# learningmatter-mit/surface-sampling

Measured on AMD Instinct MI355X. Metric: MC energy-evaluations/sec (SrTiO3(001) ~250-atom slabs, 3-model PaiNN ensemble E+F incl. neighbor list), higher is better.
Workload: dtype f32 via fp16x2-split MFMA (3 products), fp32 accumulate; neighbor decisions f64; 1 GPU; SrTiO3(001) PaiNN x3, 256 batched independent chains per GPU (BASELINE configs[3]), 248-272 atoms/chain; chains_per_gpu=256, atoms_per_gpu=66503, edges_per_gpu=2747786, slots_per_gpu=2836316, models=3, streams_per_gpu=2, parallelism=one GPU, no collective

## Files before the change

### include/vssr_eval.h

```cpp
#ifndef VSSR_EVAL_H
#define VSSR_EVAL_H

#include <stddef.h>
#include <stdint.h>

#ifdef __cplusplus
extern "C" {
#endif

#define VSSR_ABI_VERSION 1

enum {
    VSSR_OK = 0,
    VSSR_E_BADARG = -1,
    VSSR_E_DEVICE = -2,
    VSSR_E_CAPACITY = -3,
    VSSR_E_NOMEM = -4,
    VSSR_E_STATE = -5
};

enum {
    VSSR_WANT_ENERGY = 1u,
    VSSR_WANT_FORCES = 2u,
    VSSR_WANT_STD = 4u,
// ... 67 lines not shown
    float maxstep;
} vssr_bfgs_params;
int vssr_batch_relax_bfgs(vssr_handle *h, const vssr_bfgs_params *params, const uint8_t *fixed, uint32_t want,
                          double *pos_out, int32_t *n_steps, uint8_t *converged);

int vssr_batch_traj_configure(vssr_handle *h, int32_t record_interval);
int vssr_batch_traj_read(vssr_handle *h, int32_t cap_records, int32_t *n_records, double *pos, float *forces, double *energy,
                         int32_t *max_records);

typedef struct {
    int32_t max_iter;
    int32_t max_eval;
    double etol, ftol;
    double dmax;
} vssr_cg_params;
int vssr_batch_relax_cg(vssr_handle *h, const vssr_cg_params *params, const uint8_t *fixed, uint32_t want,
                        double *pos_out, int32_t *n_iter, int32_t *n_eval, int32_t *stop_reason);

int vssr_profile_enable(vssr_handle *h, int enable);
int vssr_profile_reset(vssr_handle *h);
int vssr_profile_read(vssr_handle *h, int32_t cap, const char **names, int64_t *launches,
                      double *total_ms, int32_t *n_out);
int vssr_batch_stats(vssr_handle *h, int64_t *n_atoms, int64_t *n_edges, int64_t *n_slots);
int vssr_batch_neighbors(vssr_handle *h, int64_t cap, int32_t *ei, int32_t *ej, int32_t *eS,
                         float *er, int64_t *n_edges);
int vssr_batch_device_results(vssr_handle *h, const float **energy, const float **energy_std);
int vssr_batch_device_results_f64(vssr_handle *h, const double **energy, const double **energy_std);
int vssr_batch_energy_f64(vssr_handle *h, double *energy, double *energy_std, double *energy_models);
int vssr_batch_embedding(vssr_handle *h, int32_t model, float *dst, int64_t cap, int64_t *n_out);
int vssr_batch_saturated(vssr_handle *h, uint8_t *flags, int32_t *n_flagged);
int vssr_batch_stress(vssr_handle *h, double *stress, double *stress_std);
int vssr_device_context(vssr_handle *h, int32_t *device, void **stream, const int32_t **overflow_flag);
int vssr_debug_capacity(vssr_handle *h, int32_t slots_per_atom, int32_t tight, int32_t *n_regrows);
int vssr_batch_relax_counts(vssr_handle *h, int64_t *lockstep_evaluations, int64_t *chain_evaluations);
int vssr_debug_read(vssr_handle *h, const char *name, int32_t model, float *dst, int64_t cap,
                    int64_t *n_out);

typedef struct {
    int32_t nrho, nr;
    double drho, dr, cutoff;
} vssr_eam_grid;
int vssr_eam_create(int32_t device, const vssr_eam_grid *grid, const double *frho, const double *zr, const double *rhor,
                    vssr_handle **out);
int vssr_eam_create_alloy(int32_t device, int32_t n_elem, int32_t fs, const vssr_eam_grid *grid, const double *frho,
                          const double *rhor, const double *z2r, vssr_handle **out);
int vssr_eam_eval_batch(vssr_handle *h, int32_t n_cfg, const int32_t *n_atoms, const int32_t *type, const double *pos,
                        const double *cell, const uint8_t *pbc, uint32_t want, vssr_out *out, double *energy_f64,
                        double *energy_atoms_f64, double *forces_f64);

int vssr_tersoff_create(int32_t device, int32_t n_types, const double *params, vssr_handle **out);
int vssr_tersoff_create_from_text(int32_t device, const char *param_text, int32_t n_species, const char *const *species,
                                  vssr_handle **out);
int vssr_tersoff_eval_batch(vssr_handle *h, int32_t n_cfg, const int32_t *n_atoms,
                            const int32_t *type, const double *pos, const double *cell,
                            const uint8_t *pbc, uint32_t want, vssr_out *out,
                            double *energy_f64 , double *energy_atoms_f64,
                            double *forces_f64);

int vssr_sw_create(int32_t device, int32_t n_types, const double *params, vssr_handle **out);
int vssr_sw_create_from_text(int32_t device, const char *param_text, int32_t n_species, const char *const *species,
                             vssr_handle **out);
int vssr_sw_eval_batch(vssr_handle *h, int32_t n_cfg, const int32_t *n_atoms, const int32_t *type, const double *pos,
                       const double *cell, const uint8_t *pbc, uint32_t want, vssr_out *out, double *energy_f64,
                       double *energy_atoms_f64, double *forces_f64);

typedef struct {
// ... 76 lines not shown
```

### surface-sampling_amd/backend.py

```python

from __future__ import annotations

import ctypes as C
import importlib.util
import os
import sys

import numpy as np

_HERE = os.path.dirname(os.path.abspath(__file__))
LIB_PATH = os.environ.get("VSSR_EVAL_LIB") or os.path.join(_HERE, "libvssr_eval.so")

WANT_ENERGY, WANT_FORCES, WANT_STD, WANT_PER_MODEL, WANT_PER_ATOM = 1, 2, 4, 8, 16
WANT_ALL = WANT_ENERGY | WANT_FORCES | WANT_STD | WANT_PER_MODEL | WANT_PER_ATOM

EXPORTS = (
    "vssr_abi_version", "vssr_create", "vssr_destroy", "vssr_last_error", "vssr_eval", "vssr_eval_batch",
    "vssr_batch_upload", "vssr_batch_set_positions", "vssr_batch_run", "vssr_batch_download",
    "vssr_synchronize", "vssr_profile_enable", "vssr_profile_reset", "vssr_profile_read",
    "vssr_batch_stats", "vssr_batch_neighbors", "vssr_debug_read", "vssr_tersoff_create",
    "vssr_tersoff_eval_batch", "vssr_batch_relax_fire", "vssr_batch_relax_bfgs", "vssr_debug_capacity",
    "vssr_batch_device_results", "vssr_eam_create", "vssr_eam_eval_batch",
    "vssr_tersoff_create_from_text", "vssr_batch_relax_cg", "vssr_batch_saturated",
    "vssr_batch_embedding", "vssr_batch_traj_configure", "vssr_batch_traj_read",
    "vssr_device_context", "vssr_batch_stress", "vssr_batch_energy_f64", "vssr_batch_device_results_f64",
    "vssr_batch_relax_counts", "vssr_sw_create", "vssr_sw_create_from_text", "vssr_sw_eval_batch",
    "vssr_gmm_create", "vssr_gmm_score_rows", "vssr_gmm_score_batch", "vssr_eam_create_alloy",
    "vssr_gmm_fit_create", "vssr_gmm_fit_append_rows", "vssr_gmm_fit_append_batch", "vssr_gmm_fit_clear",
    "vssr_gmm_fit_set_init", "vssr_gmm_fit_run", "vssr_gmm_fit_params", "vssr_gmm_fit_scorer",
    "vssr_cluster_create", "vssr_cluster_append_rows", "vssr_cluster_append_batch", "vssr_cluster_clear", "vssr_cluster_pca",
    "vssr_cluster_pca_params", "vssr_cluster_projected", "vssr_cluster_set_points", "vssr_cluster_linkage",
)


class BackendError(RuntimeError):
    pass


class PainnConfig(C.Structure):
    _fields_ = [
        ("struct_size", C.c_uint32), ("device", C.c_int32), ("n_models", C.c_int32),
        ("weights", C.POINTER(C.POINTER(C.c_float))), ("weights_len", C.c_uint64),
        ("feat_dim", C.c_int32), ("n_rbf", C.c_int32), ("num_conv", C.c_int32), ("n_embed", C.c_int32),
        ("readout_hidden", C.c_int32), ("cutoff", C.c_float), ("excl_vol", C.c_int32),
        ("excl_power", C.c_int32), ("excl_sigma", C.c_float), ("model_units_per_ev", C.c_double),
        ("offset_per_z", C.POINTER(C.c_double)), ("offset_const", C.c_double),
    ]


class FireParams(C.Structure):
    _fields_ = [("max_steps", C.c_int32), ("fmax", C.c_float), ("dt", C.c_float), ("maxstep", C.c_float),
                ("dtmax", C.c_float), ("finc", C.c_float), ("fdec", C.c_float), ("astart", C.c_float),
                ("fa", C.c_float), ("nmin", C.c_int32)]

    @classmethod
    def default(cls, max_steps=20, fmax=0.01):
        return cls(int(max_steps), float(fmax), 0.1, 0.2, 1.0, 1.1, 0.5, 0.1, 0.99, 5)


class EamGrid(C.Structure):
    _fields_ = [("nrho", C.c_int32), ("nr", C.c_int32), ("drho", C.c_double), ("dr", C.c_double), ("cutoff", C.c_double)]


class CgParams(C.Structure):
# ... 139 lines not shown
    L.vssr_eam_eval_batch.argtypes = L.vssr_tersoff_eval_batch.argtypes
    L.vssr_sw_create.restype = C.c_int
    L.vssr_sw_create.argtypes = [C.c_int32, C.c_int32, dp, C.POINTER(vp)]
    L.vssr_sw_create_from_text.restype = C.c_int
    L.vssr_sw_create_from_text.argtypes = [C.c_int32, C.c_char_p, C.c_int32, C.POINTER(C.c_char_p), C.POINTER(vp)]
    L.vssr_sw_eval_batch.restype = C.c_int
    L.vssr_sw_eval_batch.argtypes = L.vssr_tersoff_eval_batch.argtypes
    L.vssr_batch_relax_fire.restype = C.c_int
    L.vssr_batch_relax_fire.argtypes = [vp, C.POINTER(FireParams), u8p, C.c_uint32, dp, ip, u8p]
    L.vssr_batch_relax_bfgs.restype = C.c_int
    L.vssr_batch_relax_bfgs.argtypes = [vp, C.POINTER(BfgsParams), u8p, C.c_uint32, dp, ip, u8p]
    L.vssr_batch_device_results.restype = C.c_int
    L.vssr_batch_device_results.argtypes = [vp, C.POINTER(vp), C.POINTER(vp)]
    L.vssr_batch_device_results_f64.restype = C.c_int
    L.vssr_batch_device_results_f64.argtypes = [vp, C.POINTER(vp), C.POINTER(vp)]
    L.vssr_batch_relax_counts.restype = C.c_int
    L.vssr_batch_relax_counts.argtypes = [vp, i64p, i64p]
    L.vssr_batch_energy_f64.restype = C.c_int
    L.vssr_batch_energy_f64.argtypes = [vp, dp, dp, dp]
    L.vssr_batch_traj_configure.restype = C.c_int
    L.vssr_batch_traj_configure.argtypes = [vp, C.c_int32]
    L.vssr_batch_traj_read.restype = C.c_int
    L.vssr_batch_traj_read.argtypes = [vp, C.c_int32, ip, dp, fp, dp, ip]
    L.vssr_batch_embedding.restype = C.c_int
    L.vssr_batch_embedding.argtypes = [vp, C.c_int32, fp, C.c_int64, i64p]
    L.vssr_batch_saturated.restype = C.c_int
    L.vssr_batch_saturated.argtypes = [vp, u8p, ip]
    L.vssr_batch_stress.restype = C.c_int
    L.vssr_batch_stress.argtypes = [vp, dp, dp]
    L.vssr_device_context.restype = C.c_int
    L.vssr_device_context.argtypes = [vp, ip, C.POINTER(vp), C.POINTER(vp)]
    L.vssr_debug_capacity.restype = C.c_int
    L.vssr_debug_capacity.argtypes = [vp, C.c_int32, C.c_int32, ip]
    L.vssr_gmm_create.restype = C.c_int
    L.vssr_gmm_create.argtypes = [C.POINTER(GmmConfig), C.POINTER(vp)]
    L.vssr_gmm_score_rows.restype = C.c_int
    L.vssr_gmm_score_rows.argtypes = [vp, C.c_int64, dp, dp, dp]
    L.vssr_gmm_score_batch.restype = C.c_int
    L.vssr_gmm_score_batch.argtypes = [vp, vp, C.c_int32, C.c_int32, C.c_int32, dp, dp]
    L.vssr_gmm_fit_create.restype = C.c_int
    L.vssr_gmm_fit_create.argtypes = [C.POINTER(GmmFitConfig), C.POINTER(vp)]
    L.vssr_gmm_fit_append_rows.restype = C.c_int
    L.vssr_gmm_fit_append_rows.argtypes = [vp, C.c_int64, dp]
    L.vssr_gmm_fit_append_batch.restype = C.c_int
    L.vssr_gmm_fit_append_batch.argtypes = [vp, vp, C.c_int32, C.c_int32]
    L.vssr_gmm_fit_clear.restype = C.c_int
    L.vssr_gmm_fit_clear.argtypes = [vp]
    L.vssr_gmm_fit_set_init.restype = C.c_int
    L.vssr_gmm_fit_set_init.argtypes = [vp, dp, dp, dp, C.POINTER(C.c_int32)]
    L.vssr_gmm_fit_run.restype = C.c_int
    L.vssr_gmm_fit_run.argtypes = [vp, C.POINTER(GmmFitResult)]
    L.vssr_gmm_fit_params.restype = C.c_int
    L.vssr_gmm_fit_params.argtypes = [vp, dp, dp, dp, dp]
    L.vssr_gmm_fit_scorer.restype = C.c_int
    L.vssr_gmm_fit_scorer.argtypes = [vp, C.c_double, C.POINTER(vp)]
    L.vssr_cluster_create.restype = C.c_int
    L.vssr_cluster_create.argtypes = [C.POINTER(ClusterConfig), C.POINTER(vp)]
    L.vssr_cluster_append_rows.restype = C.c_int
    L.vssr_cluster_append_rows.argtypes = [vp, C.c_int64, dp]
    L.vssr_cluster_append_batch.restype = C.c_int
    L.vssr_cluster_append_batch.argtypes = [vp, vp, C.c_int32]
    L.vssr_cluster_clear.restype = C.c_int
    L.vssr_cluster_clear.argtypes = [vp]
    L.vssr_cluster_pca.restype = C.c_int
    L.vssr_cluster_pca.argtypes = [vp, C.POINTER(ClusterPcaResult)]
    L.vssr_cluster_pca_params.restype = C.c_int
# ... 614 lines not shown
```

### surface-sampling_amd/csrc/painn_edge_mfma.hip

```cpp
#include "vssr_internal.h"

#ifdef EDGE_PHASE_TIMING
__device__ unsigned long long g_edge_phase[16];
#define EPH_INIT unsigned long long eph_acc[8] = {0, 0, 0, 0, 0, 0, 0, 0}, eph_t = wall_clock64();
#define EPH(k) { __builtin_amdgcn_sched_barrier(0); const unsigned long long eph_n = wall_clock64(); eph_acc[k] += eph_n - eph_t; eph_t = eph_n; __builtin_amdgcn_sched_barrier(0); }
#define EPH_FLUSH(base) if ((threadIdx.x & 63) == 0) { for (int q_ = 0; q_ < 8; ++q_) atomicAdd(&g_edge_phase[(base) + q_], eph_acc[q_]); }
extern "C" int vssr_debug_edge_phases(unsigned long long *out, int reset) {
    if (hipMemcpyFromSymbol(out, HIP_SYMBOL(g_edge_phase), sizeof(unsigned long long) * 16) != hipSuccess) return -1;
    if (reset) { unsigned long long z[16] = {}; if (hipMemcpyToSymbol(HIP_SYMBOL(g_edge_phase), z, sizeof(z)) != hipSuccess) return -1; }
    return 0;
}
#else
#define EPH_INIT
#define EPH(k)
#define EPH_FLUSH(base)
#endif

#ifndef SUB16_WAVES
#define SUB16_WAVES 12
#endif

namespace vssr {

typedef float f32x4 __attribute__((ext_vector_type(4)));
// ... 98 lines not shown
                split2(Wd[(size_t)row * 20 + kq + 4 * t], p2);
                wh[t] = p2[0]; wl[t] = p2[1];
            }
            split2(bd[row], bp);
            const unsigned bias = kq == 1 ? bp[1] : kq == 3 ? 0u : bp[0];
            const unsigned a1[8] = {wh[0], wh[1], wh[2], wh[3], wh[4], bias, wl[0], wl[1]};
            const unsigned a2[8] = {wl[2], wl[3], wl[4], wh[4], wh[0], wh[1], wh[2], wh[3]};
            unsigned *o = dst + ((size_t)row * 4 + kq) * 8;
            for (int q = 0; q < 4; ++q) {
                o[q] = a1[2 * q] | (a1[2 * q + 1] << 16);
                o[4 + q] = a2[2 * q] | (a2[2 * q + 1] << 16);
            }
        }
}

#ifndef STAGE_BATCH
#define STAGE_BATCH 4
#endif

template <int N> struct FeatVec { typedef float type __attribute__((ext_vector_type(N))); };
struct FeatVec1 {
    float v;
    __device__ __forceinline__ float operator[](int) const { return v; }
};
template <> struct FeatVec<1> { typedef FeatVec1 type; };

template <int NF>
struct EdgeGeo {
    static_assert(NF == 4 || NF == 2 || NF == 1, "16-, 8- or 4-feature slices");
    static constexpr int FS = 4 * NF;
    static constexpr int NSLICE = F / FS;
    static constexpr int NSEC = 3;
    static constexpr int NT = NF == 4 ? 3 : NF == 2 ? 2 : 1;
    static constexpr int NSEG = 6;
    static constexpr int ROW = NSEG * FS + 4;
    static constexpr int ROWB = FS * 4 + 4;
    __host__ __device__ static constexpr int row_section(int T, int i) {
        return NF == 4 ? T : NF == 1 ? ((i & 3) < 3 ? (i & 3) : -1) : (2 * T + ((i & 3) >> 1) < 3 ? 2 * T + ((i & 3) >> 1) : -1);
    }
    __host__ __device__ static constexpr int row_feature(int i) { return NF == 4 ? i : NF == 1 ? (i >> 2) : 2 * (i >> 2) + (i & 1); }
};
template <int NF> __device__ __forceinline__ constexpr int sec_tile(int sec) { return NF == 4 ? sec : NF == 1 ? 0 : sec >> 1; }
template <int NF> __device__ __forceinline__ constexpr int sec_reg(int sec, int r) { return NF == 4 ? r : NF == 1 ? sec : 2 * (sec & 1) + r; }

template <int NF, bool SLDS>
size_t edge_fwd_lds_bytes_t(int max_atoms) {
    return sizeof(float) * ((size_t)max_atoms * (EdgeGeo<NF>::ROW + (SLDS ? EdgeGeo<NF>::FS : 0)) + 4);
}

typedef float f32x2v __attribute__((ext_vector_type(2)));
#if defined(__HIP_DEVICE_COMPILE__)
typedef __attribute__((address_space(3))) const float lds_cfloat;
__device__ __forceinline__ lds_cfloat *lds_base(const float *p) { return (lds_cfloat *)p; }
__device__ __forceinline__ lds_cfloat *lds_row(lds_cfloat *base, int row, int row_floats) {
    return base + __umul24((unsigned)row, (unsigned)row_floats);
}
__device__ __forceinline__ f32x4 lds_read4(lds_cfloat *p) { return *reinterpret_cast<__attribute__((address_space(3))) const f32x4 *>(p); }
__device__ __forceinline__ f32x2v lds_read2(lds_cfloat *p) { return *reinterpret_cast<__attribute__((address_space(3))) const f32x2v *>(p); }
#else
typedef const float lds_cfloat;
__host__ __device__ inline lds_cfloat *lds_base(const float *p) { return p; }
__host__ __device__ inline lds_cfloat *lds_row(lds_cfloat *base, int row, int row_floats) { return base + row * row_floats; }
__host__ __device__ inline f32x4 lds_read4(lds_cfloat *p) { return *reinterpret_cast<const f32x4 *>(p); }
__host__ __device__ inline f32x2v lds_read2(lds_cfloat *p) { return *reinterpret_cast<const f32x2v *>(p); }
#endif

__device__ __forceinline__ float quad_sum(float x) {
    x += __builtin_bit_cast(float, __builtin_amdgcn_update_dpp(0, __builtin_bit_cast(int, x), 0xB1, 0xF, 0xF, true));
// ... 84 lines not shown
template <bool ALIASED> struct EdgeOut { typedef float *__restrict__ ptr; };
template <> struct EdgeOut<true> { typedef float *ptr; };

template <int NF, bool SLDS, int WAVES, bool SUB = false>
__global__ void __launch_bounds__(64 * WAVES) __attribute__((amdgpu_waves_per_eu((SUB && NF == 4) ? WAVES / 4 : 4, (SUB && NF == 4) ? WAVES / 4 : 4)))
k_edge_fwd_mfma(int N, int l, const ModelW *__restrict__ MW, GraphView G, const int *__restrict__ counters,
                int zero_slot, int n_models, int max_atoms, const int *__restrict__ list, int n_list,
                const float *__restrict__ s_in, const float *__restrict__ v_in, const float *__restrict__ phi,
                typename EdgeOut<SUB>::ptr s_msg, typename EdgeOut<SUB>::ptr v_msg, const int4 *__restrict__ bundle_tab,
                const int *__restrict__ n_entries_tab, int pass, int chunk_max) {
    using LY = EdgeGeo<NF>;
    constexpr int FS = LY::FS, NSLICE = LY::NSLICE, NT = LY::NT, EDGE_THREADS = 64 * WAVES;
    static_assert(!SUB || !SLDS, "the sub-range form takes its residuals from memory");
    extern __shared__ __attribute__((aligned(16))) float tile[];
    if (counters[2]) return;
    int t;
    const int b = chain_of_workgroup(G, list, n_list, NSLICE * n_models, t);
    if (b < 0) return;
    const int fs = t % NSLICE, m = t / NSLICE;
    const int a0 = G.cfg_start[b], Nc = G.cfg_start[b + 1] - a0;
    const size_t mN = (size_t)m * N;
    const int tid = threadIdx.x;
    int lo = 0, ns = Nc;
    if constexpr (SUB) {
        if (pass >= sub_passes(Nc, chunk_max)) return;
        const int chunk = sub_chunk(Nc, chunk_max);
        lo = pass * chunk;
        ns = min(chunk, Nc - lo);
    }
    const float *res_s = (SUB && pass) ? s_msg : s_in, *res_v = (SUB && pass) ? v_msg : v_in;

    float *s_tile = tile + (size_t)max_atoms * LY::ROW;
    {
        constexpr int Q4 = FS / 4;
        constexpr int PER_ATOM = (LY::NSEG + (SLDS ? 1 : 0)) * Q4;
        const int total = ns * PER_ATOM;
        if constexpr (SUB) {
            for (int k = tid; k < LY::ROW; k += EDGE_THREADS) tile[(size_t)ns * LY::ROW + k] = 0.f;
        }
        auto src_of = [&](int idx) -> const float * {
            int atom = idx / PER_ATOM, rem = idx - atom * PER_ATOM, seg = rem / Q4, q4 = rem % Q4;
            const size_t ga = mN + a0 + lo + atom;
            if (seg == LY::NSEG) return s_in + ga * F + fs * FS + q4 * 4;
            if (seg < 3) return phi + ga * F3 + seg * F + fs * FS + q4 * 4;
            return v_in + (ga * 3 + (seg - 3)) * F + fs * FS + q4 * 4;
        };
        auto put = [&](int idx, const float4 &val) {
            int atom = idx / PER_ATOM, rem = idx - atom * PER_ATOM, seg = rem / Q4, q4 = rem % Q4;
            if (seg == LY::NSEG) {
                *reinterpret_cast<float4 *>(s_tile + atom * FS + q4 * 4) = val;
            } else {
                float *dst = tile + atom * LY::ROW + (q4 * 4) * LY::NSEG + seg;
                dst[0] = val.x; dst[LY::NSEG] = val.y; dst[2 * LY::NSEG] = val.z; dst[3 * LY::NSEG] = val.w;
            }
        };
        for (int base = tid; base < total; base += STAGE_BATCH * EDGE_THREADS) {
            float4 v4[STAGE_BATCH];
#pragma unroll
            for (int u = 0; u < STAGE_BATCH; ++u) {
                const int idx = min(base + u * EDGE_THREADS, total - 1);
                v4[u] = *reinterpret_cast<const float4 *>(src_of(idx));
            }
#pragma unroll
            for (int u = 0; u < STAGE_BATCH; ++u)
                if (base + u * EDGE_THREADS < total) put(base + u * EDGE_THREADS, v4[u]);
        }
    }
    __syncthreads();

    const int lane = tid & 63, wave = tid >> 6, p = lane & 15, fq = lane >> 4, e = p & 3;
    const LayerW &W = MW[m].layer[l];
    u32x4 wA[NT][2];
#pragma unroll
    for (int T = 0; T < NT; ++T) {
        const int sec = LY::row_section(T, p);
        const int row = max(sec, 0) * F + fs * FS + LY::row_feature(p);
        const u32x4 *wsrc = reinterpret_cast<const u32x4 *>(W.wd16) + ((size_t)row * 4 + fq) * 2;
#pragma unroll
        for (int i3 = 0; i3 < 2; ++i3) wA[T][i3] = sec < 0 ? (u32x4){0u, 0u, 0u, 0u} : gload_u32x4(wsrc + i3);
    }

    BundleWalk<EDGE_THREADS / 64> bw;
    int n_entries = Nc;
    if constexpr (SUB) {
        if (pass) n_entries = n_entries_tab[(size_t)(pass - 1) * G.n_cfg + b];
    }
    bw.init((SUB ? bundle_tab : G.bundle) + a0, n_entries, __builtin_amdgcn_readfirstlane(wave), p >> 2);
    if (bw.nj == 0) return;
#ifdef ABL_STAGE_ONLY
    if (bw.nj > 0) return;
#endif
    float ds[NF], dvx[NF], dvy[NF], dvz[NF];
#pragma unroll
    for (int r = 0; r < NF; ++r) { ds[r] = 0.f; dvx[r] = 0.f; dvy[r] = 0.f; dvz[r] = 0.f; }
    const int fcol = fs * FS + NF * fq;
    typedef typename FeatVec<NF>::type fres;
    fres sres_cur, sres_nxt, vres_cur[SUB ? 3 : 1];
    auto load_residual = [&](int cc) {
        return *reinterpret_cast<const fres *>(res_s + (mN + a0 + min(max(cc, 0), Nc - 1)) * F + fcol);
    };
    auto load_residual_v = [&](int cc, int x) {
        return *reinterpret_cast<const fres *>(res_v + ((mN + a0 + min(max(cc, 0), Nc - 1)) * 3 + x) * F + fcol);
    };
    if (!SLDS) { sres_cur = load_residual(bw.cur.x); sres_nxt = load_residual(bw.nxt.x); }
    if constexpr (SUB) {
#pragma unroll
        for (int x = 0; x < 3; ++x) vres_cur[x] = load_residual_v(bw.cur.x, x);
    }

    const u32x4 *rho_lane = reinterpret_cast<const u32x4 *>(G.rho16) + fq * 4 + e;
    const int zero_quad = (zero_slot + 1) / 4 - 1;

    u32x4 rq[2][2];
    auto fetch = [&](int buf, int quad_first_slot, bool valid) {
#ifdef ABL_TABLE_L2
        const u32x4 *rp = rho_lane + (size_t)(valid ? ((quad_first_slot >> 2) & 511) : zero_quad) * 32;
#else
        const u32x4 *rp = rho_lane + (size_t)(unsigned)(valid ? (quad_first_slot >> 2) : zero_quad) * 32;
#endif
        rq[buf][0] = rp[0]; rq[buf][1] = rp[16];
    };
    {
        bool v0, v1;
        const int q0 = bw.quad_ahead(0, v0), q1 = bw.quad_ahead(1, v1);
        fetch(0, q0, v0);
        __builtin_amdgcn_sched_barrier(0);
        fetch(1, q1, v1);
    }

    auto flush_bundle = [&]() {
        quad_sum_n<NF>(ds); quad_sum_n<NF>(dvx); quad_sum_n<NF>(dvy); quad_sum_n<NF>(dvz);
        const int c = bw.cur.x;
        if (e == 0 && c >= 0) {
            const size_t ga = mN + a0 + c;
            float so[NF], xo[NF], yo[NF], zo[NF];
            const float *sr = s_tile + c * FS + NF * fq;
            const float *vc = tile + c * LY::ROW + (NF * fq) * LY::NSEG;
#pragma unroll
            for (int r = 0; r < NF; ++r) {
                so[r] = ds[r] + (SLDS ? sr[r] : sres_cur[r]);
                xo[r] = dvx[r] + (SUB ? vres_cur[0][r] : vc[r * LY::NSEG + 3]);
                yo[r] = dvy[r] + (SUB ? vres_cur[SUB ? 1 : 0][r] : vc[r * LY::NSEG + 4]);
                zo[r] = dvz[r] + (SUB ? vres_cur[SUB ? 2 : 0][r] : vc[r * LY::NSEG + 5]);
            }
            store_feat<NF>(s_msg + ga * F + fcol, so);
            store_feat<NF>(v_msg + (ga * 3 + 0) * F + fcol, xo);
            store_feat<NF>(v_msg + (ga * 3 + 1) * F + fcol, yo);
            store_feat<NF>(v_msg + (ga * 3 + 2) * F + fcol, zo);
        }
#pragma unroll
        for (int r = 0; r < NF; ++r) { ds[r] = 0.f; dvx[r] = 0.f; dvy[r] = 0.f; dvz[r] = 0.f; }
    };

    lds_cfloat *trow = lds_base(tile) + (NF * fq) * LY::NSEG;
    EPH_INIT
    EPH(0)
    while (bw.j < bw.nj) {
#pragma unroll
        for (int ph = 0; ph < 2; ++ph) {
            arrival_fence(rq[ph][0], rq[ph][1]);
            EPH(1)
#ifdef ABL_LDS_BCAST
            const int jn = (int)(rq[ph][0][3] >> 16) & 1;
#else
            int jn = (int)rq[ph][1][3];
            if constexpr (SUB) {
                const unsigned jl = (unsigned)(jn - lo);
                jn = jl < (unsigned)ns ? (int)jl : ns;
            }
#endif
            if (bw.t == bw.Lc) {
                flush_bundle();
                bw.advance();
                if (!SLDS) {
                    sres_cur = sres_nxt;
                    __builtin_amdgcn_sched_barrier(0);
                    sres_nxt = load_residual(bw.nxt.x);
                    if constexpr (SUB) {
#pragma unroll
                        for (int x = 0; x < 3; ++x) vres_cur[x] = load_residual_v(bw.cur.x, x);
                    }
                }
                EPH(2)
            }
            float tv[NF * LY::NSEG];
            {
                if constexpr ((NF * LY::NSEG) % 4 == 0) {
                    lds_cfloat *row = lds_row(trow, jn, LY::ROW);
#pragma unroll
                    for (int q = 0; q < NF * LY::NSEG / 4; ++q) {
                        const f32x4 t4 = lds_read4(row + 4 * q);
                        tv[4 * q] = t4[0]; tv[4 * q + 1] = t4[1]; tv[4 * q + 2] = t4[2]; tv[4 * q + 3] = t4[3];
                    }
                } else {
                    lds_cfloat *row = lds_row(trow, jn, LY::ROW);
#pragma unroll
                    for (int q = 0; q < NF * LY::NSEG / 2; ++q) {
                        const f32x2v t2 = lds_read2(row + 2 * q);
                        tv[2 * q] = t2[0]; tv[2 * q + 1] = t2[1];
                    }
                }
            }
            float ux, uy, uz, invd_unused;
            slot_scalars(take_u(rq[ph][1][2]), ux, uy, uz, invd_unused);
            u32x4 rb2 = dense_b2(rq[ph][0], rq[ph][1]);
            mfma_pre_fence(rq[ph][0], rb2);
            EPH(3)
            f32x4 acc[NT];
            {
                const u32x4 (*wp[NT])[2], *bp1[NT], *bp2[NT];
#pragma unroll
                for (int s2 = 0; s2 < NT; ++s2) { wp[s2] = &wA[s2]; bp1[s2] = &rq[ph][0]; bp2[s2] = &rb2; }
                filter_tiles_dense<NT>(wp, bp1, bp2, acc);
            }
            __builtin_amdgcn_sched_barrier(0);
            EPH(4)
            auto message = [&](int r) {
                const float *tr = tv + r * LY::NSEG;
                const float wa = acc[sec_tile<NF>(0)][sec_reg<NF>(0, r)], wb = acc[sec_tile<NF>(1)][sec_reg<NF>(1, r)],
                            wc = acc[sec_tile<NF>(2)][sec_reg<NF>(2, r)];
                ds[r] = fmaf(tr[1], wb, ds[r]);
                const float mc = tr[2] * wc, ma = tr[0] * wa;
                dvx[r] = fmaf(mc, ux, dvx[r]); dvy[r] = fmaf(mc, uy, dvy[r]); dvz[r] = fmaf(mc, uz, dvz[r]);
                dvx[r] = fmaf(ma, tr[3], dvx[r]);
                dvy[r] = fmaf(ma, tr[4], dvy[r]);
                dvz[r] = fmaf(ma, tr[5], dvz[r]);
            };
            message(0);
            bool nv;
            int nq = bw.quad_ahead(2, nv);
            mfma_load_fence(nq, ds[0], dvx[0], dvy[0]);
            EPH(5)
            fetch(ph, nq, nv);
            __builtin_amdgcn_sched_barrier(0);
#ifdef ABL_HALF_VALU
#pragma unroll
            for (int r = 1; r < NF / 2; ++r) message(r);
#else
#pragma unroll
            for (int r = 1; r < NF; ++r) message(r);
#endif
            ++bw.t;
            EPH(6)
        }
    }
    EPH_FLUSH(0)
}

template <int NF, int WAVES>
constexpr int cen_floats() { return WAVES * 4 * 4 * 6 * NF; }
template <int NF, int WAVES>
#ifdef ABL_LDS_FORCE
size_t edge_bwd_lds_bytes_t(int max_atoms) { return sizeof(float) * ((size_t)max_atoms * EdgeGeo<NF>::ROWB + cen_floats<NF, WAVES>()) + 24 * (size_t)max_atoms + 32; }
#else
size_t edge_bwd_lds_bytes_t(int max_atoms) { return sizeof(float) * ((size_t)max_atoms * EdgeGeo<NF>::ROWB + cen_floats<NF, WAVES>()); }
#endif

template <int NF, bool FIRST, int WAVES, bool SUB = false>
__global__ void __launch_bounds__(64 * WAVES) __attribute__((amdgpu_waves_per_eu(2, 2)))
// ... 342 lines not shown
            }
            ++bw.t;
            EPH(7)
        }
    }
    EPH_FLUSH(8)
#ifdef ABL_LDS_FORCE
    __syncthreads();
    {
        unsigned long long *dst = reinterpret_cast<unsigned long long *>(gb) + (size_t)3 * a0;
        for (int i = tid; i < 3 * Nc; i += BWD_THREADS) dst[i] = facc[i];
    }
#endif
}



int edge_mfma_init(vssr_handle *h) {
#define SET_LDS(K) VSSR_HIP(h, hipFuncSetAttribute((const void *)(K), hipFuncAttributeMaxDynamicSharedMemorySize, 160 * 1024))
    SET_LDS((k_edge_fwd_mfma<4, true, 16>)); SET_LDS((k_edge_fwd_mfma<4, false, 16>)); SET_LDS((k_edge_fwd_mfma<2, false, 16>)); SET_LDS((k_edge_fwd_mfma<2, false, 16, true>)); SET_LDS((k_edge_fwd_mfma<4, false, SUB16_WAVES, true>));
    SET_LDS((k_edge_fwd_mfma<4, true, 8>)); SET_LDS((k_edge_fwd_mfma<4, true, 4>)); SET_LDS((k_edge_fwd_mfma<1, false, 16>));
    SET_LDS((k_edge_bwd_mfma<1, true, 4>)); SET_LDS((k_edge_bwd_mfma<1, false, 4>));
    SET_LDS((k_edge_bwd_mfma<1, true, 8>)); SET_LDS((k_edge_bwd_mfma<1, false, 8>));
    SET_LDS((k_edge_bwd_mfma<4, true, 4>)); SET_LDS((k_edge_bwd_mfma<4, false, 4>));
    SET_LDS((k_edge_bwd_mfma<2, true, 4>)); SET_LDS((k_edge_bwd_mfma<2, false, 4>));
    SET_LDS((k_edge_bwd_mfma<4, true, 8>)); SET_LDS((k_edge_bwd_mfma<4, false, 8>));
    SET_LDS((k_edge_bwd_mfma<4, true, 8, true>)); SET_LDS((k_edge_bwd_mfma<4, false, 8, true>));
    SET_LDS((k_edge_bwd_mfma<2, true, 8>)); SET_LDS((k_edge_bwd_mfma<2, false, 8>));
#undef SET_LDS
    return VSSR_OK;
}

int edge_class_of(int n_atoms) {
    if (edge_fwd_lds_bytes_t<4, true>(n_atoms) <= 160 * 1024) return EDGE_CLASS_FS16;
    if (edge_fwd_lds_bytes_t<4, false>(n_atoms) <= 160 * 1024) return EDGE_CLASS_FS16M;
    if (edge_fwd_lds_bytes_t<2, false>(n_atoms) <= 160 * 1024) return EDGE_CLASS_FS8;
    if (edge_fwd_lds_bytes_t<1, false>(n_atoms) <= 160 * 1024) return EDGE_CLASS_FS4;
    return EDGE_CLASS_GATHER;
}
int edge_bclass_of(int n_atoms) {
    const int fwd = edge_class_of(n_atoms);
    if (fwd == EDGE_CLASS_GATHER) return EDGE_BCLASS_GATHER;
    if (edge_bwd_lds_bytes_t<4, 8>(n_atoms) <= 160 * 1024) return EDGE_BCLASS_FS16;
    if (edge_bwd_lds_bytes_t<2, 8>(n_atoms) <= 160 * 1024) return EDGE_BCLASS_FS8;
    return EDGE_BCLASS_FS4;
}
int edge_class_groups(int bcls) { return edge_bclass_slices(bcls); }
static_assert(edge_bclass_slices(EDGE_BCLASS_FS16) == EdgeGeo<4>::NSLICE && edge_bclass_slices(EDGE_BCLASS_FS8) == EdgeGeo<2>::NSLICE &&
              edge_bclass_slices(EDGE_BCLASS_FS4) == EdgeGeo<1>::NSLICE, "slices per reverse class");

void launch_edge_bwd_mfma(hipStream_t st, int cls, int N, const int *list, int n_list, int M, int l, int layer_first, int max_atoms,
                          const ModelW *MW, const GraphView &G, const int *counters, int zero_slot,
                          const float *v_in, const float *phi, const float *sbar_msg, const float *vbar_msg,
                          float *phibar, float *vbar_in, float *gbar, long long gbar_stride, int n_groups, int group_off, int rec,
                          const int4 *bundle_sub, int sub_chunk) {
    if (n_list <= 0) return;
    if (cls == EDGE_BCLASS_FS16P) {
        const int chunk_max = sub_chunk, passes = sub_passes(max_atoms, chunk_max), staged = min(chunk_max, max_atoms) + 1;
        const int *n_entries = reinterpret_cast<const int *>(bundle_sub + (size_t)SUB_MAX_PASSES * N);
        for (int pass = 0; pass < passes; ++pass) {
#define LAUNCH_BWD_SUB(FIRST)                                                                                                    \
    hipLaunchKernelGGL((k_edge_bwd_mfma<4, FIRST, 8, true>), dim3(((n_list + 7) / 8) * 8 * EdgeGeo<4>::NSLICE * M), dim3(64 * 8),   \
                       (edge_bwd_lds_bytes_t<4, 8>(staged)), st, N, l, MW, G, counters, zero_slot, M, staged, list, n_list, v_in, phi, \
                       sbar_msg, vbar_msg, phibar, vbar_in, gbar, gbar_stride, n_groups, group_off, rec, bundle_sub + (size_t)pass * N, \
                       n_entries, pass, chunk_max)
            if (layer_first) LAUNCH_BWD_SUB(true); else LAUNCH_BWD_SUB(false);
#undef LAUNCH_BWD_SUB
        }
        return;
    }
// ... 20 lines not shown
                          const float *phi, float *s_msg, float *v_msg, const int4 *bundle_sub, int sub_width, int sub_chunk) {
    if (n_list <= 0) return;
#define LAUNCH_FWD(NF, SLDS, WAVES)                                                                                                \
    hipLaunchKernelGGL((k_edge_fwd_mfma<NF, SLDS, WAVES>), dim3(((n_list + 7) / 8) * 8 * EdgeGeo<NF>::NSLICE * M), dim3(64 * WAVES), \
                       (edge_fwd_lds_bytes_t<NF, SLDS>(max_atoms)), st, N, l, MW, G, counters, zero_slot, M, max_atoms, list, n_list, \
                       s_in, v_in, phi, s_msg, v_msg, (const int4 *)nullptr, (const int *)nullptr, 0, 0)
    if (cls == EDGE_CLASS_FS16) {
        const size_t lds = edge_fwd_lds_bytes_t<4, true>(max_atoms);
        const long long wgs = (long long)n_list * EdgeGeo<4>::NSLICE * M;
        if (4 * lds <= 160 * 1024 && wgs > 4 * 256) LAUNCH_FWD(4, true, 4);
        else if (2 * lds <= 160 * 1024 && wgs > 2 * 256) LAUNCH_FWD(4, true, 8);
        else LAUNCH_FWD(4, true, 16);
    } else if (cls == EDGE_CLASS_FS16M) LAUNCH_FWD(4, false, 16);
    else if (cls == EDGE_CLASS_FS8) LAUNCH_FWD(2, false, 16);
    else if (bundle_sub) {
        const int chunk_max = sub_chunk, passes = sub_passes(max_atoms, chunk_max);
        const int staged = min(chunk_max, max_atoms) + 1;
        const int *n_entries = reinterpret_cast<const int *>(bundle_sub + (size_t)SUB_MAX_PASSES * N);
        for (int pass = 0; pass < passes; ++pass) {
            if (sub_width == 16)
                hipLaunchKernelGGL((k_edge_fwd_mfma<4, false, SUB16_WAVES, true>), dim3(((n_list + 7) / 8) * 8 * EdgeGeo<4>::NSLICE * M), dim3(64 * SUB16_WAVES),
                                   (edge_fwd_lds_bytes_t<4, false>(staged)), st, N, l, MW, G, counters, zero_slot, M, staged, list, n_list,
                                   s_in, v_in, phi, s_msg, v_msg, bundle_sub + (size_t)pass * N, n_entries, pass, chunk_max);
            else
                hipLaunchKernelGGL((k_edge_fwd_mfma<2, false, 16, true>), dim3(((n_list + 7) / 8) * 8 * EdgeGeo<2>::NSLICE * M), dim3(64 * 16),
                                   (edge_fwd_lds_bytes_t<2, false>(staged)), st, N, l, MW, G, counters, zero_slot, M, staged, list, n_list,
                                   s_in, v_in, phi, s_msg, v_msg, bundle_sub + (size_t)pass * N, n_entries, pass, chunk_max);
        }
    } else LAUNCH_FWD(1, false, 16);
#undef LAUNCH_FWD
}

}
```

### surface-sampling_amd/csrc/vssr_internal.h

```cpp
#pragma once

#include <hip/hip_runtime.h>

#include <cstdint>
#include <cstdio>
#include <cstdlib>
#include <cstring>
#include <string>
#include <vector>

#include "../../include/vssr_eval.h"

namespace vssr {

constexpr int F = 128;
constexpr int F3 = 3 * F;
constexpr int MAX_LAYERS = 4;
constexpr int MAX_MODELS = 8;
constexpr int RB_MAX = 24;
constexpr int NODE_TILE = 8;
constexpr int L0_MAX_SPECIES = 8;

struct LayerW {
    const float *W1, *W1t, *b1;
// ... 389 lines not shown
void launch_msg_mlp_mfma(hipStream_t st, int N, int M, int l, const ActiveView &av, const ModelW *MW, const float *s_in,
                         float *phi);
void launch_msg_mlp_bwd_mfma(hipStream_t st, int N, int M, int l, const ActiveView &av, const ModelW *MW, const float *s_in,
                             const float *phibar, const float *sbar_msg, float *sbar_in);
void launch_update_fwd_mfma(hipStream_t st, int N, int M, int l, const ActiveView &av, const ModelW *MW, const float *s_msg,
                            const float *v_msg, float *s_out, float *v_out, float *phi_next, void *save);
size_t update_save_bytes(int N, int M);
bool readout_mfma_supported(int hidden);
void launch_readout_mfma(hipStream_t st, int N, int M, const ActiveView &av, const ModelW *MW, const float *s, const float *e_excl,
                         float *e_atom);
void launch_update_bwd_mfma(hipStream_t st, int N, int M, int l, int mode, int vbar_is_zero, const ActiveView &av, const ModelW *MW,
                            const float *s_msg, const float *v_msg, const float *sbar_src, const float *vbar,
                            const float *s_next, const float *phibar, const float *e_excl, float *e_atom,
                            float *sbar_msg, float *vbar_msg, const void *save);
void pack_mfma_tiles16(const float *Wsrc, int rows, int K, unsigned *dst );
void build_wd16(const float *Wd, const float *bd, unsigned *dst );
void l0_build_tables(const float *blob_embed, const float *W1, const float *b1, const float *W2, const float *b2,
                     const float *Wd, const float *bd, int n_embed, float *A, float *At);
void l0_pack_tables(const float *A, int n_embed, unsigned *A16, unsigned *At16);
size_t l0_packed_dwords(int n_embed);
int l0_mfma_init(vssr_handle *h);
int l0_run_forward(vssr_handle *h, const GraphView &G, float *s_msg, float *v_msg);
int l0_run_reverse(vssr_handle *h, const GraphView &G, int first_write, int fresh_mfma, const float *sbar_msg, const float *vbar_msg,
                   float4 *gbar, long long gbar_stride, int n_groups);
int edge_mfma_init(vssr_handle *h);
enum { EDGE_CLASS_FS16 = 0, EDGE_CLASS_FS16M = 1, EDGE_CLASS_FS8 = 2, EDGE_CLASS_FS4 = 3, EDGE_CLASS_GATHER = 4, EDGE_CLASSES = 5,
       EDGE_MFMA_CLASSES = 4 };
enum { EDGE_BCLASS_FS16 = 0, EDGE_BCLASS_FS8 = 1, EDGE_BCLASS_FS4 = 2, EDGE_BCLASS_FS16P = 3, EDGE_BCLASS_GATHER = 4, EDGE_BCLASSES = 5,
       EDGE_MFMA_BCLASSES = 4 };
__host__ __device__ constexpr int edge_bclass_slices(int c) { return (c == EDGE_BCLASS_FS16 || c == EDGE_BCLASS_FS16P) ? 8 : c == EDGE_BCLASS_FS8 ? 16 : c == EDGE_BCLASS_FS4 ? 32 : 1; }
int edge_bclass_of(int n_atoms);
int edge_class_of(int n_atoms);
constexpr int SUB_MAX_PASSES = 4;
__host__ __device__ constexpr int sub_chunk_max(int width) { return width == 16 ? 400 : 784; }
__host__ __device__ constexpr int sub_chunk_max_bwd() { return 550; }
__host__ __device__ constexpr int sub_passes(int n_atoms, int chunk_max) { return (n_atoms + chunk_max - 1) / chunk_max; }
__host__ __device__ constexpr int sub_chunk(int n_atoms, int chunk_max) { return (n_atoms + sub_passes(n_atoms, chunk_max) - 1) / sub_passes(n_atoms, chunk_max); }
int edge_class_groups(int cls);
void launch_edge_bwd_mfma(hipStream_t st, int cls, int N, const int *list, int n_list, int M, int l, int layer_first, int max_atoms,
                          const ModelW *MW, const GraphView &G, const int *counters, int zero_slot,
                          const float *v_in, const float *phi, const float *sbar_msg, const float *vbar_msg,
                          float *phibar, float *vbar_in, float *gbar, long long gbar_stride, int n_groups, int group_off, int rec,
                          const int4 *bundle_sub, int sub_chunk);
void launch_edge_fwd_mfma(hipStream_t st, int cls, int N, const int *list, int n_list, int M, int l, int max_atoms, const ModelW *MW,
                          const GraphView &G, const int *counters, int zero_slot, const float *s_in, const float *v_in,
                          const float *phi, float *s_msg, float *v_msg, const int4 *bundle_sub, int sub_width, int sub_chunk);

}
```

Before: 24680 evaluations/s.

## Precombine phi*v into staged LDS rows and shrink edge forward tile to five words

The forward edge MFMA kernel now stages per-neighbor rows holding phi_b, phi_c and phi_a*v premultiplied, which cuts the row from six words per feature to five (padded to six only for width 4). That lowers LDS footprint and per-edge reads and saves a multiply per message. Sub-chunk limits are now derived from the LDS budget, so more atoms fit per pass or a wider class can be chosen. The flush path also changes so each lane writes one output component (s, vx, vy or vz) keyed by its lane index instead of lane 0 writing all four, with residuals loaded per lane. A debug export for the edge class is added.

```diff
diff --git a/include/vssr_eval.h b/include/vssr_eval.h
--- a/include/vssr_eval.h
+++ b/include/vssr_eval.h
@@ -123,6 +123,7 @@
 int vssr_batch_stress(vssr_handle *h, double *stress, double *stress_std);
 int vssr_device_context(vssr_handle *h, int32_t *device, void **stream, const int32_t **overflow_flag);
 int vssr_debug_capacity(vssr_handle *h, int32_t slots_per_atom, int32_t tight, int32_t *n_regrows);
+int vssr_debug_edge_class(int32_t n_atoms, int32_t *fwd_class, int64_t *lds_bytes, int64_t *lds_limit);
 int vssr_batch_relax_counts(vssr_handle *h, int64_t *lockstep_evaluations, int64_t *chain_evaluations);
 int vssr_debug_read(vssr_handle *h, const char *name, int32_t model, float *dst, int64_t cap,
                     int64_t *n_out);
diff --git a/surface-sampling_amd/backend.py b/surface-sampling_amd/backend.py
--- a/surface-sampling_amd/backend.py
+++ b/surface-sampling_amd/backend.py
@@ -30,6 +30,7 @@
     "vssr_gmm_fit_set_init", "vssr_gmm_fit_run", "vssr_gmm_fit_params", "vssr_gmm_fit_scorer",
     "vssr_cluster_create", "vssr_cluster_append_rows", "vssr_cluster_append_batch", "vssr_cluster_clear", "vssr_cluster_pca",
     "vssr_cluster_pca_params", "vssr_cluster_projected", "vssr_cluster_set_points", "vssr_cluster_linkage",
+    "vssr_debug_edge_class",
 )
 
 
@@ -235,6 +236,8 @@
     L.vssr_device_context.argtypes = [vp, ip, C.POINTER(vp), C.POINTER(vp)]
     L.vssr_debug_capacity.restype = C.c_int
     L.vssr_debug_capacity.argtypes = [vp, C.c_int32, C.c_int32, ip]
+    L.vssr_debug_edge_class.restype = C.c_int
+    L.vssr_debug_edge_class.argtypes = [C.c_int32, ip, i64p, i64p]
     L.vssr_gmm_create.restype = C.c_int
     L.vssr_gmm_create.argtypes = [C.POINTER(GmmConfig), C.POINTER(vp)]
     L.vssr_gmm_score_rows.restype = C.c_int
diff --git a/surface-sampling_amd/csrc/painn_edge_mfma.hip b/surface-sampling_amd/csrc/painn_edge_mfma.hip
--- a/surface-sampling_amd/csrc/painn_edge_mfma.hip
+++ b/surface-sampling_amd/csrc/painn_edge_mfma.hip
@@ -154,8 +154,10 @@
     static constexpr int NSLICE = F / FS;
     static constexpr int NSEC = 3;
     static constexpr int NT = NF == 4 ? 3 : NF == 2 ? 2 : 1;
-    static constexpr int NSEG = 6;
-    static constexpr int ROW = NSEG * FS + 4;
+    static constexpr int NSEG = edge_fwd_row_words;
+    static constexpr int FSTR = edge_fwd_feature_stride(FS);
+    static constexpr int ROW = edge_fwd_row_floats(FS);
+    static_assert(ROW == FSTR * FS + 4 && ROW % 4 == 0 && (NF * FSTR) % 2 == 0, "staged rows: 16-byte rows, 8-byte lane blocks");
     static constexpr int ROWB = FS * 4 + 4;
     __host__ __device__ static constexpr int row_section(int T, int i) {
         return NF == 4 ? T : NF == 1 ? ((i & 3) < 3 ? (i & 3) : -1) : (2 * T + ((i & 3) >> 1) < 3 ? 2 * T + ((i & 3) >> 1) : -1);
@@ -306,38 +308,37 @@
 
     float *s_tile = tile + (size_t)max_atoms * LY::ROW;
     {
-        constexpr int Q4 = FS / 4;
-        constexpr int PER_ATOM = (LY::NSEG + (SLDS ? 1 : 0)) * Q4;
-        const int total = ns * PER_ATOM;
+        constexpr int Q4 = FS / 4, QW = 4 * LY::FSTR;
+        const int total = ns * Q4;
         if constexpr (SUB) {
             for (int k = tid; k < LY::ROW; k += EDGE_THREADS) tile[(size_t)ns * LY::ROW + k] = 0.f;
         }
-        auto src_of = [&](int idx) -> const float * {
-            int atom = idx / PER_ATOM, rem = idx - atom * PER_ATOM, seg = rem / Q4, q4 = rem % Q4;
+        for (int idx = tid; idx < total; idx += EDGE_THREADS) {
+            const int atom = idx / Q4, q4 = idx - atom * Q4;
             const size_t ga = mN + a0 + lo + atom;
-            if (seg == LY::NSEG) return s_in + ga * F + fs * FS + q4 * 4;
-            if (seg < 3) return phi + ga * F3 + seg * F + fs * FS + q4 * 4;
-            return v_in + (ga * 3 + (seg - 3)) * F + fs * FS + q4 * 4;
-        };
-        auto put = [&](int idx, const float4 &val) {
-            int atom = idx / PER_ATOM, rem = idx - atom * PER_ATOM, seg = rem / Q4, q4 = rem % Q4;
-            if (seg == LY::NSEG) {
-                *reinterpret_cast<float4 *>(s_tile + atom * FS + q4 * 4) = val;
-            } else {
-                float *dst = tile + atom * LY::ROW + (q4 * 4) * LY::NSEG + seg;
-                dst[0] = val.x; dst[LY::NSEG] = val.y; dst[2 * LY::NSEG] = val.z; dst[3 * LY::NSEG] = val.w;
-            }
-        };
-        for (int base = tid; base < total; base += STAGE_BATCH * EDGE_THREADS) {
-            float4 v4[STAGE_BATCH];
-#pragma unroll
-            for (int u = 0; u < STAGE_BATCH; ++u) {
-                const int idx = min(base + u * EDGE_THREADS, total - 1);
-                v4[u] = *reinterpret_cast<const float4 *>(src_of(idx));
-            }
-#pragma unroll
-            for (int u = 0; u < STAGE_BATCH; ++u)
-                if (base + u * EDGE_THREADS < total) put(base + u * EDGE_THREADS, v4[u]);
+            const int col = fs * FS + q4 * 4;
+            f32x4 ph[3], vv[3], sq;
+#pragma unroll
+            for (int sec = 0; sec < 3; ++sec) ph[sec] = *reinterpret_cast<const f32x4 *>(phi + ga * F3 + sec * F + col);
+#pragma unroll
+            for (int x = 0; x < 3; ++x) vv[x] = *reinterpret_cast<const f32x4 *>(v_in + (ga * 3 + x) * F + col);
+            if constexpr (SLDS) sq = *reinterpret_cast<const f32x4 *>(s_in + ga * F + col);
+            float w[QW];
+#pragma unroll
+            for (int k = 0; k < 4; ++k) {
+                const float a = ph[0][k];
+                w[k * LY::FSTR + 0] = ph[1][k];
+                w[k * LY::FSTR + 1] = ph[2][k];
+                w[k * LY::FSTR + 2] = a * vv[0][k];
+                w[k * LY::FSTR + 3] = a * vv[1][k];
+                w[k * LY::FSTR + 4] = a * vv[2][k];
+                if constexpr (LY::FSTR > LY::NSEG) w[k * LY::FSTR + 5] = 0.f;
+            }
+            float *dst = tile + atom * LY::ROW + q4 * QW;
+#pragma unroll
+            for (int q = 0; q < QW / 4; ++q)
+                *reinterpret_cast<f32x4 *>(dst + 4 * q) = (f32x4){w[4 * q], w[4 * q + 1], w[4 * q + 2], w[4 * q + 3]};
+            if constexpr (SLDS) *reinterpret_cast<f32x4 *>(s_tile + atom * FS + q4 * 4) = sq;
         }
     }
     __syncthreads();
@@ -369,18 +370,14 @@
     for (int r = 0; r < NF; ++r) { ds[r] = 0.f; dvx[r] = 0.f; dvy[r] = 0.f; dvz[r] = 0.f; }
     const int fcol = fs * FS + NF * fq;
     typedef typename FeatVec<NF>::type fres;
-    fres sres_cur, sres_nxt, vres_cur[SUB ? 3 : 1];
-    auto load_residual = [&](int cc) {
-        return *reinterpret_cast<const fres *>(res_s + (mN + a0 + min(max(cc, 0), Nc - 1)) * F + fcol);
+    fres res_cur;
+    const int res_mul = e == 0 ? 1 : 3, res_add = e == 0 ? 0 : e - 1;
+    auto residual_row = [&](const float *sp, const float *vp, int cc) -> const float * {
+        const float *base = e == 0 ? sp : vp;
+        return base + ((mN + a0 + cc) * res_mul + res_add) * F + fcol;
     };
-    auto load_residual_v = [&](int cc, int x) {
-        return *reinterpret_cast<const fres *>(res_v + ((mN + a0 + min(max(cc, 0), Nc - 1)) * 3 + x) * F + fcol);
-    };
-    if (!SLDS) { sres_cur = load_residual(bw.cur.x); sres_nxt = load_residual(bw.nxt.x); }
-    if constexpr (SUB) {
-#pragma unroll
-        for (int x = 0; x < 3; ++x) vres_cur[x] = load_residual_v(bw.cur.x, x);
-    }
+    auto load_residual = [&](int cc) { return *reinterpret_cast<const fres *>(residual_row(res_s, res_v, min(max(cc, 0), Nc - 1))); };
+    res_cur = load_residual(bw.cur.x);
 
     const u32x4 *rho_lane = reinterpret_cast<const u32x4 *>(G.rho16) + fq * 4 + e;
     const int zero_quad = (zero_slot + 1) / 4 - 1;
@@ -405,28 +402,22 @@
     auto flush_bundle = [&]() {
         quad_sum_n<NF>(ds); quad_sum_n<NF>(dvx); quad_sum_n<NF>(dvy); quad_sum_n<NF>(dvz);
         const int c = bw.cur.x;
-        if (e == 0 && c >= 0) {
-            const size_t ga = mN + a0 + c;
-            float so[NF], xo[NF], yo[NF], zo[NF];
-            const float *sr = s_tile + c * FS + NF * fq;
-            const float *vc = tile + c * LY::ROW + (NF * fq) * LY::NSEG;
+        if (c >= 0) {
+            float o[NF];
 #pragma unroll
             for (int r = 0; r < NF; ++r) {
-                so[r] = ds[r] + (SLDS ? sr[r] : sres_cur[r]);
-                xo[r] = dvx[r] + (SUB ? vres_cur[0][r] : vc[r * LY::NSEG + 3]);
-                yo[r] = dvy[r] + (SUB ? vres_cur[SUB ? 1 : 0][r] : vc[r * LY::NSEG + 4]);
-                zo[r] = dvz[r] + (SUB ? vres_cur[SUB ? 2 : 0][r] : vc[r * LY::NSEG + 5]);
-            }
-            store_feat<NF>(s_msg + ga * F + fcol, so);
-            store_feat<NF>(v_msg + (ga * 3 + 0) * F + fcol, xo);
-            store_feat<NF>(v_msg + (ga * 3 + 1) * F + fcol, yo);
-            store_feat<NF>(v_msg + (ga * 3 + 2) * F + fcol, zo);
+                float sum = dvz[r], res = res_cur[r];
+                sum = e == 2 ? dvy[r] : sum; sum = e == 1 ? dvx[r] : sum; sum = e == 0 ? ds[r] : sum;
+                if constexpr (SLDS) { const float sl = s_tile[c * FS + NF * fq + r]; res = e == 0 ? sl : res; }
+                o[r] = sum + res;
+            }
+            store_feat<NF>(const_cast<float *>(residual_row(s_msg, v_msg, c)), o);
         }
 #pragma unroll
         for (int r = 0; r < NF; ++r) { ds[r] = 0.f; dvx[r] = 0.f; dvy[r] = 0.f; dvz[r] = 0.f; }
     };
 
-    lds_cfloat *trow = lds_base(tile) + (NF * fq) * LY::NSEG;
+    lds_cfloat *trow = lds_base(tile) + (NF * fq) * LY::FSTR;
     EPH_INIT
     EPH(0)
     while (bw.j < bw.nj) {
@@ -446,33 +437,28 @@
             if (bw.t == bw.Lc) {
                 flush_bundle();
                 bw.advance();
-                if (!SLDS) {
-                    sres_cur = sres_nxt;
-                    __builtin_amdgcn_sched_barrier(0);
-                    sres_nxt = load_residual(bw.nxt.x);
-                    if constexpr (SUB) {
-#pragma unroll
-                        for (int x = 0; x < 3; ++x) vres_cur[x] = load_residual_v(bw.cur.x, x);
-                    }
-                }
+                res_cur = load_residual(bw.cur.x);
                 EPH(2)
             }
             float tv[NF * LY::NSEG];
             {
+                lds_cfloat *row = lds_row(trow, jn, LY::ROW);
                 if constexpr ((NF * LY::NSEG) % 4 == 0) {
-                    lds_cfloat *row = lds_row(trow, jn, LY::ROW);
 #pragma unroll
                     for (int q = 0; q < NF * LY::NSEG / 4; ++q) {
                         const f32x4 t4 = lds_read4(row + 4 * q);
                         tv[4 * q] = t4[0]; tv[4 * q + 1] = t4[1]; tv[4 * q + 2] = t4[2]; tv[4 * q + 3] = t4[3];
                     }
-                } else {
-                    lds_cfloat *row = lds_row(trow, jn, LY::ROW);
+                } else if constexpr ((NF * LY::NSEG) % 2 == 0) {
 #pragma unroll
                     for (int q = 0; q < NF * LY::NSEG / 2; ++q) {
                         const f32x2v t2 = lds_read2(row + 2 * q);
                         tv[2 * q] = t2[0]; tv[2 * q + 1] = t2[1];
                     }
+                } else {
+                    static_assert(NF == 1 && LY::NSEG == 5, "one feature per lane");
+                    const f32x2v t0 = lds_read2(row), t1 = lds_read2(row + 2);
+                    tv[0] = t0[0]; tv[1] = t0[1]; tv[2] = t1[0]; tv[3] = t1[1]; tv[4] = row[4];
                 }
             }
             float ux, uy, uz, invd_unused;
@@ -493,12 +479,12 @@
                 const float *tr = tv + r * LY::NSEG;
                 const float wa = acc[sec_tile<NF>(0)][sec_reg<NF>(0, r)], wb = acc[sec_tile<NF>(1)][sec_reg<NF>(1, r)],
                             wc = acc[sec_tile<NF>(2)][sec_reg<NF>(2, r)];
-                ds[r] = fmaf(tr[1], wb, ds[r]);
-                const float mc = tr[2] * wc, ma = tr[0] * wa;
+                ds[r] = fmaf(tr[0], wb, ds[r]);
+                const float mc = tr[1] * wc;
                 dvx[r] = fmaf(mc, ux, dvx[r]); dvy[r] = fmaf(mc, uy, dvy[r]); dvz[r] = fmaf(mc, uz, dvz[r]);
-                dvx[r] = fmaf(ma, tr[3], dvx[r]);
-                dvy[r] = fmaf(ma, tr[4], dvy[r]);
-                dvz[r] = fmaf(ma, tr[5], dvz[r]);
+                dvx[r] = fmaf(wa, tr[2], dvx[r]);
+                dvy[r] = fmaf(wa, tr[3], dvy[r]);
+                dvz[r] = fmaf(wa, tr[4], dvz[r]);
             };
             message(0);
             bool nv;
@@ -907,10 +893,10 @@
 }
 
 int edge_class_of(int n_atoms) {
-    if (edge_fwd_lds_bytes_t<4, true>(n_atoms) <= 160 * 1024) return EDGE_CLASS_FS16;
-    if (edge_fwd_lds_bytes_t<4, false>(n_atoms) <= 160 * 1024) return EDGE_CLASS_FS16M;
-    if (edge_fwd_lds_bytes_t<2, false>(n_atoms) <= 160 * 1024) return EDGE_CLASS_FS8;
-    if (edge_fwd_lds_bytes_t<1, false>(n_atoms) <= 160 * 1024) return EDGE_CLASS_FS4;
+    if (edge_fwd_lds_bytes_t<4, true>(n_atoms) <= EDGE_LDS_BYTES) return EDGE_CLASS_FS16;
+    if (edge_fwd_lds_bytes_t<4, false>(n_atoms) <= EDGE_LDS_BYTES) return EDGE_CLASS_FS16M;
+    if (edge_fwd_lds_bytes_t<2, false>(n_atoms) <= EDGE_LDS_BYTES) return EDGE_CLASS_FS8;
+    if (edge_fwd_lds_bytes_t<1, false>(n_atoms) <= EDGE_LDS_BYTES) return EDGE_CLASS_FS4;
     return EDGE_CLASS_GATHER;
 }
 int edge_bclass_of(int n_atoms) {
@@ -997,3 +983,14 @@
 }
 
 }
+
+extern "C" int vssr_debug_edge_class(int32_t n_atoms, int32_t *fwd_class, int64_t *lds_bytes, int64_t *lds_limit) {
+    if (n_atoms < 0 || !fwd_class || !lds_bytes || !lds_limit) return VSSR_E_BADARG;
+    *fwd_class = vssr::edge_class_of(n_atoms);
+    lds_bytes[0] = (int64_t)vssr::edge_fwd_lds_bytes_t<4, true>(n_atoms);
+    lds_bytes[1] = (int64_t)vssr::edge_fwd_lds_bytes_t<4, false>(n_atoms);
+    lds_bytes[2] = (int64_t)vssr::edge_fwd_lds_bytes_t<2, false>(n_atoms);
+    lds_bytes[3] = (int64_t)vssr::edge_fwd_lds_bytes_t<1, false>(n_atoms);
+    *lds_limit = vssr::EDGE_LDS_BYTES;
+    return VSSR_OK;
+}
diff --git a/surface-sampling_amd/csrc/vssr_internal.h b/surface-sampling_amd/csrc/vssr_internal.h
--- a/surface-sampling_amd/csrc/vssr_internal.h
+++ b/surface-sampling_amd/csrc/vssr_internal.h
@@ -445,7 +445,11 @@
 int edge_bclass_of(int n_atoms);
 int edge_class_of(int n_atoms);
 constexpr int SUB_MAX_PASSES = 4;
-__host__ __device__ constexpr int sub_chunk_max(int width) { return width == 16 ? 400 : 784; }
+constexpr int edge_fwd_row_words = 5;
+constexpr int EDGE_LDS_BYTES = 160 * 1024;
+__host__ __device__ constexpr int edge_fwd_feature_stride(int width) { return width == 4 ? edge_fwd_row_words + 1 : edge_fwd_row_words; }
+__host__ __device__ constexpr int edge_fwd_row_floats(int width) { return edge_fwd_feature_stride(width) * width + 4; }
+__host__ __device__ constexpr int sub_chunk_max(int width) { return (EDGE_LDS_BYTES / 4 - 4) / edge_fwd_row_floats(width) - 1; }
 __host__ __device__ constexpr int sub_chunk_max_bwd() { return 550; }
 __host__ __device__ constexpr int sub_passes(int n_atoms, int chunk_max) { return (n_atoms + chunk_max - 1) / chunk_max; }
 __host__ __device__ constexpr int sub_chunk(int n_atoms, int chunk_max) { return (n_atoms + sub_passes(n_atoms, chunk_max) - 1) / sub_passes(n_atoms, chunk_max); }
```

Result: no change. 24750 evaluations/s, median of 6 (+0.3%).
